# invesalius/invesalius3

Measured on AMD Instinct MI355X. Metric: Mvoxel/s segmentation + Mtriangles/s marching-cubes, 512^3 int16, 1/2/4/8 GPU, higher is better.
Workload: dtype i16; 1 GPU; configs[1]: 512x512x512 int16 per GPU, threshold(226..3071) + 26-neighbour region-grow + marching-cubes(mask@127); global_voxels=134217728, parallelism=z-slab x1, collectives=none, overlap=none

## Files before the change

### invesalius3_amd/csrc/k_mc.hip

```cpp
#include <algorithm>

#include "levels_write.h"
#include "mc_common.h"

#define MC_TABLE_QUAL static __device__ __attribute__((aligned(16))) const
#include "../../include/ivx_mc_tables.h"

typedef short short8_t __attribute__((ext_vector_type(8)));
typedef unsigned char uchar16_t __attribute__((ext_vector_type(16)));

using namespace ivx;

namespace {

template <typename T, int NISO>
__global__ __launch_bounds__(256) void k_mc_bits(const T *__restrict__ a, int64_t nrows_src, int64_t nx, int64_t ws,
                                                 double iso0, double iso1, uint8_t *__restrict__ bits0,
                                                 uint8_t *__restrict__ bits1) {
    constexpr int V = 16 / sizeof(T);
    constexpr int OB = V / 8;
    const int64_t cpr = ws * 64 / V;
    const int64_t total = nrows_src * cpr;
    const int64_t stride = (int64_t)gridDim.x * blockDim.x;
    const bool vec = (nx % V == 0) && (((uintptr_t)a & 15) == 0);
    if (vec && ws * 64 == nx) {
        const int64_t nchunk = nrows_src * (nx / V);
        typedef T vec_t __attribute__((ext_vector_type(V)));
        const vec_t *src = reinterpret_cast<const vec_t *>(a);
        for (int64_t t0 = ((int64_t)blockIdx.x * blockDim.x) * 4 + threadIdx.x; t0 < nchunk; t0 += stride * 4) {
            vec_t x[4];
#pragma unroll
            for (int u = 0; u < 4; u++) {
                const int64_t t = t0 + (int64_t)u * blockDim.x;
                if (t < nchunk) x[u] = __builtin_nontemporal_load(&src[t]);
            }
#pragma unroll
            for (int u = 0; u < 4; u++) {
                const int64_t t = t0 + (int64_t)u * blockDim.x;
                if (t >= nchunk) continue;
                unsigned m0 = 0, m1 = 0;
#pragma unroll
                for (int e = 0; e < V; e++) {
                    const double d = (double)(T)x[u][e];
                    m0 |= d >= iso0 ? (1u << e) : 0u;
                    if (NISO == 2) m1 |= d >= iso1 ? (1u << e) : 0u;
                }
                if (OB == 1) {
                    bits0[t] = (uint8_t)m0;
                    if (NISO == 2) bits1[t] = (uint8_t)m1;
                } else {
                    reinterpret_cast<uint16_t *>(bits0)[t] = (uint16_t)m0;
                    if (NISO == 2) reinterpret_cast<uint16_t *>(bits1)[t] = (uint16_t)m1;
                }
            }
        }
        return;
    }
    for (int64_t t = (int64_t)blockIdx.x * blockDim.x + threadIdx.x; t < total; t += stride) {
        const int64_t row = t / cpr, q = t - row * cpr;
        const int64_t x0 = q * V;
        unsigned m0 = 0, m1 = 0;
        if (x0 < nx) {
            const T *r = a + row * nx + x0;
            T v[V];
            if (vec) {
                if (sizeof(T) == 2) {
                    const short8_t c = *reinterpret_cast<const short8_t *>(r);
#pragma unroll
                    for (int e = 0; e < V; e++) v[e] = (T)c[e % 8];
                } else {
                    const uchar16_t c = *reinterpret_cast<const uchar16_t *>(r);
#pragma unroll
                    for (int e = 0; e < V; e++) v[e] = (T)c[e % 16];
                }
            } else {
#pragma unroll
                for (int e = 0; e < V; e++) v[e] = (x0 + e < nx) ? r[e] : (T)0;
            }
#pragma unroll
            for (int e = 0; e < V; e++) {
                const bool valid = vec || (x0 + e < nx);
                const double d = (double)v[e];
                m0 |= (valid && d >= iso0) ? (1u << e) : 0u;
                if (NISO == 2) m1 |= (valid && d >= iso1) ? (1u << e) : 0u;
            }
        }
        const int64_t ob = (row * ws * 8) + q * OB;
        if (OB == 1) {
            bits0[ob] = (uint8_t)m0;
            if (NISO == 2) bits1[ob] = (uint8_t)m1;
        } else {
            *reinterpret_cast<uint16_t *>(bits0 + ob) = (uint16_t)m0;
            if (NISO == 2) *reinterpret_cast<uint16_t *>(bits1 + ob) = (uint16_t)m1;
        }
    }
}

struct Corner8 {
    uint64_t c[8];
    uint64_t active;
};
__device__ __forceinline__ uint64_t mc_shl1(uint64_t x, uint32_t below_hi) {
    const uint32_t xl = (uint32_t)x, xh = (uint32_t)(x >> 32);
    return ((uint64_t)__builtin_amdgcn_alignbit(xh, xl, 31) << 32) | __builtin_amdgcn_alignbit(xl, below_hi, 31);
}
__device__ __forceinline__ uint64_t mc_shr1(uint64_t x, uint32_t above) {
    const uint32_t xl = (uint32_t)x, xh = (uint32_t)(x >> 32);
    return ((uint64_t)__builtin_amdgcn_alignbit(above, xh, 1) << 32) | __builtin_amdgcn_alignbit(xh, xl, 1);
}
__device__ __forceinline__ uint64_t mc_lowbits(int32_t n) {
    return n >= 64 ? ~0ull : (n <= 0 ? 0ull : ((1ull << n) - 1ull));
}
__device__ __forceinline__ Corner8 load_corners(const uint64_t *__restrict__ bits, const Geom &g, int64_t k,
                                                int64_t j, int64_t w, uint64_t pbits) {
    Corner8 r;
    const auto clampi = [](int64_t v, int64_t n) { return v >= n ? (n > 0 ? n - 1 : 0) : (v < 0 ? 0 : v); };
    const int32_t w32 = (int32_t)w, NX32 = (int32_t)g.NX, nx32 = (int32_t)g.nx, ws32 = (int32_t)g.ws;
    const uint64_t exist = mc_lowbits(NX32 - w32 * 64);
    uint64_t srcm = exist;
    if (g.pxy && w32 == 0) srcm &= ~1ull;
    srcm &= mc_lowbits(g.pxy + nx32 - w32 * 64);
    const int32_t x1 = (w32 + 1) * 64;
    const bool exist1 = x1 < NX32;
    const bool src1 = x1 - g.pxy < nx32;
    const int32_t wc = w32 >= ws32 ? (ws32 > 0 ? ws32 - 1 : 0) : w32;
    const int32_t wm = w32 - 1 >= ws32 ? (ws32 > 0 ? ws32 - 1 : 0) : (w32 - 1 < 0 ? 0 : w32 - 1);
    const int32_t wp = w32 + 1 >= ws32 ? (ws32 > 0 ? ws32 - 1 : 0) : w32 + 1;
    const int32_t ja0 = ((int32_t)g.NY - 1 - (int32_t)j) - g.pxy, ka0 = (int32_t)k - g.pb;
    const bool inner = ja0 - 1 >= 0 && ja0 < (int32_t)g.ny && ka0 >= 0 && ka0 + 1 < (int32_t)g.nz;
    if (__all(inner)) {
        const uint64_t padlo = pbits & exist & ~srcm;
        const bool use1 = exist1 && src1;
        const uint32_t nbpad = exist1 ? (uint32_t)pbits & 1u : 0u;
        const uint64_t *row = bits + (uint64_t)((uint32_t)ka0 * (uint32_t)g.ny + (uint32_t)ja0) * (uint64_t)(uint32_t)ws32;
        const uint64_t *pc = row + wc, *pa = row + (g.pxy ? wm : wp);
        const int64_t dj = -g.ws, dk = g.ny * g.ws;
        uint64_t a0[4], a1[4];
#pragma unroll
        for (int q = 0; q < 4; q++) {
            const int64_t d = ((q & 1) ? dj : 0) + ((q >> 1) ? dk : 0);
            a0[q] = pc[d];
            a1[q] = pa[d];
        }
#pragma unroll
        for (int q = 0; q < 4; q++) {
            uint64_t v0;
            uint32_t raw1;
            if (g.pxy) {
                v0 = mc_shl1(a0[q], (uint32_t)(a1[q] >> 32));
                raw1 = (uint32_t)(a0[q] >> 63);
            } else {
                v0 = a0[q];
                raw1 = (uint32_t)a1[q] & 1u;
            }
            const uint64_t lo = (v0 & srcm) | padlo;
            r.c[2 * q] = lo;
            r.c[2 * q + 1] = mc_shr1(lo, use1 ? raw1 : nbpad);
        }
    } else {
        const bool has_m = w32 - 1 >= 0 && w32 - 1 < ws32, has_c = w32 < ws32, has_p = w32 + 1 < ws32;
        uint64_t a0[4], a1[4];
        bool rin[4];
#pragma unroll
        for (int q = 0; q < 4; q++) {
            const int64_t ja = (g.NY - 1 - (j + (q & 1))) - g.pxy, ka = k + (q >> 1) - g.pb;
            rin[q] = ja >= 0 && ja < g.ny && ka >= 0 && ka < g.nz;
            const uint64_t *row = bits + (clampi(ka, g.nz) * g.ny + clampi(ja, g.ny)) * g.ws;
            a0[q] = row[wc];
            a1[q] = g.pxy ? row[wm] : row[wp];
        }
#pragma unroll
        for (int q = 0; q < 4; q++) {
            const uint64_t sc = (rin[q] && has_c) ? a0[q] : 0ull;
            uint64_t v0, raw1;
            if (g.pxy) {
                const uint64_t sm = (rin[q] && has_m) ? a1[q] : 0ull;
                v0 = (sc << 1) | (sm >> 63);
                raw1 = sc >> 63;
            } else {
                const uint64_t sp = (rin[q] && has_p) ? a1[q] : 0ull;
                v0 = sc;
                raw1 = sp & 1ull;
            }
            const uint64_t src = rin[q] ? srcm : 0ull;
            const uint64_t lo = (v0 & src) | (pbits & exist & ~src);
            const uint64_t nb = exist1 ? ((rin[q] && src1) ? raw1 : (pbits & 1ull)) : 0ull;
            r.c[2 * q] = lo;
            r.c[2 * q + 1] = (lo >> 1) | (nb << 63);
        }
    }
    uint64_t any = 0, all = ~0ull;
#pragma unroll
    for (int c = 0; c < 8; c++) {
        any |= r.c[c];
        all &= r.c[c];
    }
    r.active = any & ~all & mc_lowbits(NX32 - 1 - w32 * 64);
    return r;
}

struct McRideArgs {
    const uint16_t *reached, *inside;
    int64_t nchunks;
    uint4 *out;
    unsigned int in4, sel4;
};
template <bool RIDE, bool ALL>
__device__ __forceinline__ void mc_count_body(const uint64_t *__restrict__ bits, const Geom &g, size_t nwords, uint64_t pbits,
                                              uint16_t *__restrict__ counts, uint32_t *__restrict__ bsum, const McRideArgs &ride) {
    __shared__ uint32_t s_part[4], s_wcnt[4];
    __shared__ uint8_t s_ntri[256];
    __shared__ uint64_t s_c[256][5];
    __shared__ uint8_t s_hi[256];
    __shared__ uint16_t s_slot[256];
    const int tid = threadIdx.x, lane = tid & 63, wv = tid >> 6;
    const uint8_t ntri = MC_NTRI[tid];
    const int64_t ride_i0 = (int64_t)blockIdx.x * 1024 + tid;
    LevelsWords lw;
    if (RIDE) levels_load<ALL>(ride.reached, ride.inside, ride.nchunks, ride_i0, lw);
    auto ride_rest = [&]() {
        if (!RIDE) return;
        const int64_t stride = (int64_t)gridDim.x * 1024;
        for (int64_t i0 = ride_i0 + stride; i0 < ride.nchunks; i0 += stride) {
            LevelsWords w2;
            levels_load<ALL>(ride.reached, ride.inside, ride.nchunks, i0, w2);
            levels_store<ALL>(w2, ride.nchunks, i0, ride.out, ride.in4, ride.sel4);
        }
    };
    auto ride_store = [&]() {
#if !defined(IVX_RIDE_NO_STORES)
        if (RIDE) levels_store<ALL>(lw, ride.nchunks, ride_i0, ride.out, ride.in4, ride.sel4);
#endif
    };
    const size_t wid = (size_t)blockIdx.x * 256 + tid;
    uint64_t act = 0;
    Corner8 r;
    if (wid < nwords) {
        uint32_t k, j, w;
        mc_split_wid(g, (uint32_t)wid, k, j, w);
        r = load_corners(bits, g, (int64_t)k, (int64_t)j, (int64_t)w, pbits);
        act = r.active;
        if (!act) counts[wid] = 0;
    }
#if defined(IVX_RIDE_STORES_EARLY)
    ride_store();
#endif
    const unsigned long long am = __ballot(act != 0);
    if (lane == 0) s_wcnt[wv] = (uint32_t)__popcll(am);
    s_ntri[tid] = ntri;
    __syncthreads();
    uint32_t before = 0;
    for (int q = 0; q < wv; q++) before += s_wcnt[q];
    const uint32_t nact = s_wcnt[0] + s_wcnt[1] + s_wcnt[2] + s_wcnt[3];
#if !defined(IVX_RIDE_STORES_EARLY)
    ride_store();
#endif
#if defined(IVX_RIDE_NO_WALK)
    if (RIDE) {
        if (tid == 0) bsum[blockIdx.x] = 0;
        ride_rest();
        return;
    }
#endif
    if (!nact) {
        if (tid == 0) bsum[blockIdx.x] = 0;
        ride_rest();
        return;
    }
    if (act) {
        const uint32_t slot = before + (uint32_t)__popcll(am & ((1ull << lane) - 1ull));
        s_slot[slot] = (uint16_t)tid;
        uint32_t hi = 0;
#pragma unroll
        for (int q = 0; q < 4; q++) {
            s_c[slot][q] = r.c[2 * q];
            hi |= (uint32_t)(r.c[2 * q + 1] >> 63) << q;
        }
        s_c[slot][4] = act;
        s_hi[slot] = (uint8_t)hi;
    }
    __syncthreads();
    uint32_t n = 0;
    if ((uint32_t)tid < nact) {
        const uint64_t c0 = s_c[tid][0], c1 = s_c[tid][1], c2 = s_c[tid][2], c3 = s_c[tid][3];
        uint64_t a2 = s_c[tid][4];
        const uint32_t hi = s_hi[tid];
        while (a2) {
            const int b = __builtin_ctzll(a2);
            a2 &= a2 - 1;
            int idx;
            if (b != 63)
                idx = (int)((c0 >> b) & 3ull) | ((int)((c1 >> b) & 3ull) << 2) | ((int)((c2 >> b) & 3ull) << 4) | ((int)((c3 >> b) & 3ull) << 6);
            else
                idx = (int)(c0 >> 63) | ((int)(hi & 1u) << 1) | ((int)(c1 >> 63) << 2) | ((int)(hi >> 1 & 1u) << 3) | ((int)(c2 >> 63) << 4) |
                      ((int)(hi >> 2 & 1u) << 5) | ((int)(c3 >> 63) << 6) | ((int)(hi >> 3 & 1u) << 7);
            n += s_ntri[idx];
        }
        counts[(size_t)blockIdx.x * 256 + s_slot[tid]] = (uint16_t)n;
    }
    uint32_t s = n;
#pragma unroll
    for (int o = 32; o > 0; o >>= 1) s += __shfl_xor(s, o, 64);
    if (lane == 0) s_part[wv] = s;
    __syncthreads();
    if (tid == 0) bsum[blockIdx.x] = s_part[0] + s_part[1] + s_part[2] + s_part[3];
    ride_rest();
}
__global__ __launch_bounds__(256) void k_mc_count(const uint64_t *__restrict__ bits, Geom g, size_t nwords,
                                                  uint64_t pbits, uint16_t *__restrict__ counts,
                                                  uint32_t *__restrict__ bsum) {
    mc_count_body<false, false>(bits, g, nwords, pbits, counts, bsum, McRideArgs{});
}
template <bool ALL>
__global__ __launch_bounds__(256) void k_mc_count_write(const uint64_t *__restrict__ bits, Geom g, size_t nwords, uint64_t pbits,
                                                        uint16_t *__restrict__ counts, uint32_t *__restrict__ bsum, McRideArgs ride,
                                                        ApplyWhen when) {
    if (apply_when_skips(when)) return;
    mc_count_body<true, ALL>(bits, g, nwords, pbits, counts, bsum, ride);
}

__global__ __launch_bounds__(1024) void k_mc_scan(const uint32_t *__restrict__ bsum, size_t n,
                                                  uint64_t *__restrict__ boff, uint32_t *mb, uint32_t seq) {
    __shared__ uint64_t s_wave[16];
    __shared__ uint64_t s_carry;
    __shared__ uint32_t s_tot[64], s_exc[64];
    constexpr int RND = 4;
    const int lane = threadIdx.x & 63, wv = threadIdx.x >> 6;
    const size_t base = (size_t)blockIdx.x * (1024 * 4 * RND);
    uint64_t pre = 0;
    {
        const uint4 *b4 = reinterpret_cast<const uint4 *>(bsum);
        const size_t n4 = base / 4;
        uint64_t p0 = 0, p1 = 0, p2 = 0, p3 = 0;
        size_t i = threadIdx.x;
        for (; i + 3 * 1024 < n4; i += 4 * 1024) {
            const uint4 a = b4[i], b = b4[i + 1024], c = b4[i + 2048], d = b4[i + 3072];
            p0 += (uint64_t)a.x + a.y + a.z + a.w;
            p1 += (uint64_t)b.x + b.y + b.z + b.w;
            p2 += (uint64_t)c.x + c.y + c.z + c.w;
            p3 += (uint64_t)d.x + d.y + d.z + d.w;
        }
        for (; i < n4; i += 1024) {
            const uint4 a = b4[i];
            p0 += (uint64_t)a.x + a.y + a.z + a.w;
        }
        pre = p0 + p1 + p2 + p3;
    }
#pragma unroll
    for (int o = 32; o > 0; o >>= 1) pre += __shfl_xor(pre, o, 64);
    if (lane == 0) s_wave[wv] = pre;
    const bool al16 = ((uintptr_t)bsum & 15) == 0 && ((uintptr_t)boff & 15) == 0;
    uint32_t v[RND][4], inc[RND];
#pragma unroll
    for (int r = 0; r < RND; r++) {
        const size_t i0 = base + (size_t)r * 4096 + (size_t)threadIdx.x * 4;
        if (al16 && i0 + 3 < n) {
            const uint4 a = *reinterpret_cast<const uint4 *>(bsum + i0);
            v[r][0] = a.x; v[r][1] = a.y; v[r][2] = a.z; v[r][3] = a.w;
        } else {
#pragma unroll
            for (int q = 0; q < 4; q++) v[r][q] = i0 + q < n ? bsum[i0 + q] : 0u;
        }
    }
#pragma unroll
    for (int r = 0; r < RND; r++) {
        inc[r] = v[r][0] + v[r][1] + v[r][2] + v[r][3];
#pragma unroll
        for (int o = 1; o < 64; o <<= 1) {
            const uint32_t t = __shfl_up(inc[r], o, 64);
            if (lane >= o) inc[r] += t;
        }
        if (lane == 63) s_tot[r * 16 + wv] = inc[r];
    }
    __syncthreads();
    if (wv == 0) {
        const uint32_t t = s_tot[lane];
        uint32_t e = t;
#pragma unroll
        for (int o = 1; o < 64; o <<= 1) {
            const uint32_t u = __shfl_up(e, o, 64);
            if (lane >= o) e += u;
        }
        s_exc[lane] = e - t;
        uint64_t c = 0;
        for (int q = 0; q < 16; q++) c += s_wave[q];
        if (lane == 0) s_carry = c;
        if (lane == 63 && base + 1024 * 4 * RND >= n) {
            const uint64_t total = c + e;
            boff[n] = total;
            if (mb) {
                mb[0] = (uint32_t)total;
                mb[1] = (uint32_t)(total >> 32);
                __threadfence_system();
                __hip_atomic_store(&mb[63], seq, __ATOMIC_RELEASE, __HIP_MEMORY_SCOPE_SYSTEM);
            }
        }
    }
    __syncthreads();
    const uint64_t carry = s_carry;
#pragma unroll
    for (int r = 0; r < RND; r++) {
        const size_t i0 = base + (size_t)r * 4096 + (size_t)threadIdx.x * 4;
        const uint32_t lanesum = v[r][0] + v[r][1] + v[r][2] + v[r][3];
        const uint64_t o0 = carry + (uint64_t)(s_exc[r * 16 + wv] + inc[r] - lanesum);
        const uint64_t o1 = o0 + v[r][0], o2 = o1 + v[r][1], o3 = o2 + v[r][2];
        if (al16 && i0 + 3 < n) {
            typedef unsigned long long u64x2_t __attribute__((ext_vector_type(2)));
            u64x2_t *d = reinterpret_cast<u64x2_t *>(boff + i0);
            d[0] = u64x2_t{o0, o1};
            d[1] = u64x2_t{o2, o3};
        } else {
            if (i0 < n) boff[i0] = o0;
            if (i0 + 1 < n) boff[i0 + 1] = o1;
            if (i0 + 2 < n) boff[i0 + 2] = o2;
            if (i0 + 3 < n) boff[i0 + 3] = o3;
        }
    }
}

constexpr int MCL_CHUNK = 256;
constexpr int MCL_CELLS = 2048;
__device__ __forceinline__ uint32_t mcl_wave_scan(uint32_t v) {
    v += (uint32_t)__builtin_amdgcn_update_dpp(0, (int)v, 0x111, 0xf, 0xf, false);
    v += (uint32_t)__builtin_amdgcn_update_dpp(0, (int)v, 0x112, 0xf, 0xf, false);
    v += (uint32_t)__builtin_amdgcn_update_dpp(0, (int)v, 0x114, 0xf, 0xf, false);
    v += (uint32_t)__builtin_amdgcn_update_dpp(0, (int)v, 0x118, 0xf, 0xf, false);
    v += (uint32_t)__builtin_amdgcn_update_dpp(0, (int)v, 0x142, 0xa, 0xf, false);
    v += (uint32_t)__builtin_amdgcn_update_dpp(0, (int)v, 0x143, 0xc, 0xf, false);
    return v;
}
__global__ __launch_bounds__(256) void k_mc_list(const uint64_t *__restrict__ bits, Geom g, size_t nwords, uint64_t pbits,
                                                 const uint16_t *__restrict__ counts, const uint64_t *__restrict__ boff,
                                                 uint64_t *__restrict__ list, uint64_t max_tris) {
    __shared__ uint32_t s_wave[4], s_part[2][4];
    __shared__ uint8_t s_ntri[256];
    __shared__ uint64_t s_c[4][256];
    __shared__ uint8_t s_hi[256];
    __shared__ uint64_t s_pre[256];
    __shared__ uint16_t s_cell[MCL_CELLS];
    const int tid = threadIdx.x, lane = tid & 63, wv = tid >> 6;
    const uint8_t ntri = MC_NTRI[tid];
    const size_t wid0 = (size_t)blockIdx.x * 256;
    const uint32_t n = wid0 + tid < nwords ? (uint32_t)counts[wid0 + tid] : 0u;
    const uint64_t pos0 = boff[blockIdx.x];
    if (boff[blockIdx.x + 1] == pos0 || pos0 >= max_tris) return;
    uint64_t a2 = 0;
    if (n) {
        uint32_t k, j, w;
        mc_split_wid(g, (uint32_t)(wid0 + tid), k, j, w);
        const Corner8 r = load_corners(bits, g, (int64_t)k, (int64_t)j, (int64_t)w, pbits);
        a2 = r.active;
        uint32_t hi = 0;
#pragma unroll
        for (int q = 0; q < 4; q++) {
            s_c[q][tid] = r.c[2 * q];
            hi |= (uint32_t)(r.c[2 * q + 1] >> 63) << q;
        }
        s_hi[tid] = (uint8_t)hi;
        s_pre[tid] = ((uint64_t)k << 48) | ((uint64_t)j << 32) | ((uint64_t)w << 17);
    }
    const uint32_t pc = (uint32_t)__popcll(a2);
    const uint32_t inc = mcl_wave_scan(pc);
    if (lane == 63) s_wave[wv] = inc;
    s_ntri[tid] = ntri;
    __syncthreads();
    uint32_t ci = inc - pc;
    for (int q = 0; q < wv; q++) ci += s_wave[q];
    const uint32_t ncell = s_wave[0] + s_wave[1] + s_wave[2] + s_wave[3];
    uint64_t P = pos0;
    int par = 0;
    for (uint32_t sb = 0; sb < ncell; sb += MCL_CELLS) {
        const uint32_t se = sb + MCL_CELLS < ncell ? sb + MCL_CELLS : ncell;
        while (a2 && ci < se) {
            const int b = __builtin_ctzll(a2);
            a2 &= a2 - 1;
            s_cell[ci - sb] = (uint16_t)((tid << 6) | b);
            ci++;
        }
        __syncthreads();
        for (uint32_t cb = sb; cb < se; cb += MCL_CHUNK) {
            const uint32_t c = cb + tid;
            uint32_t nt = 0;
            uint64_t d0 = 0;
            if (c < se) {
                const uint32_t rec = s_cell[c - sb], sl = rec >> 6;
                const int b = (int)(rec & 63u);
                const uint64_t c0 = s_c[0][sl], c1 = s_c[1][sl], c2 = s_c[2][sl], c3 = s_c[3][sl];
                int idx;
                if (b != 63) {
                    idx = (int)((c0 >> b) & 3ull) | ((int)((c1 >> b) & 3ull) << 2) | ((int)((c2 >> b) & 3ull) << 4) | ((int)((c3 >> b) & 3ull) << 6);
                } else {
                    const uint32_t hi = s_hi[sl];
                    idx = (int)(c0 >> 63) | ((int)(hi & 1u) << 1) | ((int)(c1 >> 63) << 2) | ((int)(hi >> 1 & 1u) << 3) | ((int)(c2 >> 63) << 4) |
                          ((int)(hi >> 2 & 1u) << 5) | ((int)(c3 >> 63) << 6) | ((int)(hi >> 3 & 1u) << 7);
                }
                nt = s_ntri[idx];
                d0 = s_pre[sl] | ((uint64_t)b << 11) | ((uint64_t)idx << 3);
            }
            const uint32_t ti = mcl_wave_scan(nt);
            if (lane == 63) s_part[par][wv] = ti;
            __syncthreads();
            uint32_t off = ti - nt;
            for (int q = 0; q < wv; q++) off += s_part[par][q];
            const uint32_t tot = s_part[par][0] + s_part[par][1] + s_part[par][2] + s_part[par][3];
            const uint64_t p0 = P + off;
#pragma unroll
            for (uint32_t t = 0; t < MC_MAX_TRI; t++)
                if (t < nt && p0 + t < max_tris) list[p0 + t] = d0 | t;
            P += tot;
            if (P >= max_tris) return;
            par ^= 1;
        }
    }
}

template <typename T, bool LEVELS>
__device__ __forceinline__ void mc_triangle(const T *__restrict__ a, const Geom &g, const McLevels &lv, double iso,
                                            const uint8_t *s_tri, const int *s_e0, const int *s_e1, const int *s_ec, int32_t k,
                                            int32_t j, int32_t i, int idx, int rel, float *o) {
    const int32_t ka = k - (int32_t)g.pb, ja = ((int32_t)g.NY - 1 - j) - (int32_t)g.pxy;
    const int32_t ia = i - (int32_t)g.pxy;
    const bool fast = ka >= 0 && ka + 1 < (int32_t)g.nz && ja - 1 >= 0 && ja < (int32_t)g.ny && ia >= 0 &&
                      ia + 1 < (int32_t)g.nx;
    double s0[3], s1[3];
    int ec[3];
#pragma unroll
    for (int v = 0; v < 3; v++) ec[v] = s_tri[idx * 15 + 3 * rel + v];
    double ttl[3];
    if (LEVELS) {
#pragma unroll
        for (int v = 0; v < 3; v++) {
            const int c = s_ec[ec[v]];
            const int ax = c & 3, bx = (c >> 2) & 1, by = (c >> 3) & 1, bz = (c >> 4) & 1;
            const int lo = bx + 2 * by + 4 * bz;
            const bool in0 = (idx >> lo) & 1, in1 = (idx >> (lo + (1 << ax))) & 1;
            const int32_t kk = k + bz + (in1 && ax == 2), jj = j + by + (in1 && ax == 1), ii = i + bx + (in1 && ax == 0);
            const int64_t sk = kk - (int32_t)g.pb, sj = ((int32_t)g.NY - 1 - jj) - (int32_t)g.pxy, si = ii - (int32_t)g.pxy;
            const uint64_t wsel = lv.sel[(sk * g.ny + sj) * g.ws + (si >> 6)];
            ttl[v] = lv.tt[(in0 ? 2 : 0) + (int)((wsel >> (si & 63)) & 1ull)];
            ec[v] = c;
        }
    } else if (fast) {
        const T *cell = a + ((int64_t)ka * g.ny + ja) * g.nx + ia;
#pragma unroll
        for (int v = 0; v < 3; v++) {
            s0[v] = (double)cell[s_e0[ec[v]]];
            s1[v] = (double)cell[s_e1[ec[v]]];
        }
#pragma unroll
        for (int v = 0; v < 3; v++) ec[v] = s_ec[ec[v]];
    } else {
#pragma unroll
        for (int v = 0; v < 3; v++) {
            const int c = s_ec[ec[v]];
            const int ax = c & 3, bx = (c >> 2) & 1, by = (c >> 3) & 1, bz = (c >> 4) & 1;
            s0[v] = mc_at(a, g, k + bz, j + by, i + bx);
            s1[v] = mc_at(a, g, k + bz + (ax == 2), j + by + (ax == 1), i + bx + (ax == 0));
            ec[v] = c;
        }
    }
#pragma unroll
    for (int v = 0; v < 3; v++) {
        const int ax = ec[v] & 3, bx = (ec[v] >> 2) & 1, by = (ec[v] >> 3) & 1, bz = (ec[v] >> 4) & 1;
        const double tt = LEVELS ? ttl[v] : (iso - s0[v]) / (s1[v] - s0[v]);
        double p0 = (double)(i + bx - (int32_t)g.pxy);
        double p1 = (double)(j + by - (int32_t)g.yoff);
        double p2 = (double)(k + bz + g.zoff);
        if (ax == 0) p0 += tt;
        else if (ax == 1) p1 += tt;
        else p2 += tt;
        o[3 * v + 0] = (float)(g.sx * p0);
        o[3 * v + 1] = (float)(g.sy * p1);
        o[3 * v + 2] = (float)(g.sz * p2);
    }
}

template <typename T, bool LEVELS>
__global__ __launch_bounds__(256) void k_mc_emit(const T *__restrict__ a, Geom g, double iso0, double iso1,
                                                 const uint64_t *__restrict__ split_dev,
                                                 const uint64_t *__restrict__ total_dev,
                                                 const uint64_t *__restrict__ list, uint64_t cap,
                                                 float *__restrict__ tris, McLevels lv) {
    __shared__ __attribute__((aligned(16))) uint8_t s_tri[256 * 15];
    __shared__ __attribute__((aligned(16))) float s_out[256 * 9];
    const int tid = threadIdx.x;
    const uint64_t total = *total_dev, split = *split_dev;
    const uint64_t ntris = total < cap ? total : cap;
    const uint64_t T0 = (uint64_t)blockIdx.x * 256;
    if (T0 >= ntris) return;
#pragma unroll
    for (int q = 0; q < 4; q++)
        if (q * 256 + tid < 960) ((uint32_t *)s_tri)[q * 256 + tid] = ((const uint32_t *)&MC_TRI[0][0])[q * 256 + tid];
    const uint64_t T_ = T0 + tid;
    const double iso = T_ < split ? iso0 : iso1;
    __shared__ int s_e0[12], s_e1[12], s_ec[12];
    const int plane32 = (int)(g.ny * g.nx), nx32 = (int)g.nx;
    if (tid < 12) {
        int ax, bx, by, bz;
        edge_decode(tid, ax, bx, by, bz);
        const int o0 = bz * plane32 - by * nx32 + bx;
        s_e0[tid] = o0;
        s_e1[tid] = o0 + (ax == 2 ? plane32 : (ax == 1 ? -nx32 : 1));
        s_ec[tid] = ax | (bx << 2) | (by << 3) | (bz << 4);
    }
    const bool live = T_ < ntris;
    const uint64_t d = live ? list[T_] : 0ull;
    __syncthreads();
    if (live) {
        const int b = (int)(d >> 11) & 63, idx = (int)(d >> 3) & 255, rel = (int)d & 7;
        const uint32_t w = (uint32_t)(d >> 17) & 0x7fffu;
        const int32_t k = (int32_t)(d >> 48), j = (int32_t)((d >> 32) & 0xffffull);
        mc_triangle<T, LEVELS>(a, g, lv, iso, s_tri, s_e0, s_e1, s_ec, k, j, (int32_t)w * 64 + b, idx, rel, s_out + tid * 9);
    }
    __syncthreads();
    const uint32_t nt_chunk = ntris - T0 < 256 ? (uint32_t)(ntris - T0) : 256u;
    float *dst = tris + T0 * 9;
    if (nt_chunk == 256 && ((uintptr_t)tris & 15) == 0) {
        typedef float float4_t __attribute__((ext_vector_type(4)));
        float4_t *d4 = (float4_t *)dst;
        const float4_t *s4 = (const float4_t *)s_out;
        __builtin_nontemporal_store(s4[tid], &d4[tid]);
        __builtin_nontemporal_store(s4[tid + 256], &d4[tid + 256]);
        if (tid < 64) __builtin_nontemporal_store(s4[tid + 512], &d4[tid + 512]);
    } else {
        for (uint32_t f = tid; f < nt_chunk * 9; f += 256) dst[f] = s_out[f];
    }
}

template <typename T>
static int run_bits(const ivx_mc_params *p, const Geom &g, const Scratch &s, const void *a, uint8_t *b0, double iso0,
                    double iso1, hipStream_t st) {
    constexpr int V = 16 / sizeof(T);
    const int64_t nrows_src = g.nz * g.ny;
    const int64_t total = nrows_src * (g.ws * 64 / V);
    if (total == 0) return IVX_OK;
    const int64_t blocks = ivx::cdiv(total, 256 * 4);
    const int grid = (int)(blocks < 1 ? 1 : (blocks < 16384 ? blocks : 16384));
    uint8_t *b1 = b0 + s.bits_words * 8;
    if (p->niso == 2)
        hipLaunchKernelGGL((k_mc_bits<T, 2>), dim3(grid), dim3(256), 0, st, (const T *)a, nrows_src, g.nx, g.ws,
                           iso0, iso1, b0, b1);
    else
        hipLaunchKernelGGL((k_mc_bits<T, 1>), dim3(grid), dim3(256), 0, st, (const T *)a, nrows_src, g.nx, g.ws,
                           iso0, 0.0, b0, b0);
    IVX_LAUNCH_CHECK();
    return IVX_OK;
}

template <typename T>
static int run_emit(const ivx_mc_params *p, const Geom &g, const Scratch &s, const void *a, const char *scratch,
                    float *tris, int64_t max_tris, hipStream_t st, const McLevels *lv) {
    const uint64_t *boff = (const uint64_t *)(scratch + s.off_boff);
    void *d_list;
    int rc = ws_get_s(WS_MCLIST, st, (size_t)max_tris * 8 + 64, &d_list);
    if (rc) return rc;
    const size_t nb = s.nblocks * (size_t)p->niso;
    if (!mc_pieces().list_ready(scratch, d_list, max_tris))
        if ((rc = mc_queue_list(p, g, s, scratch, d_list, max_tris, st))) return rc;
    if (lv)
        hipLaunchKernelGGL((k_mc_emit<T, true>), dim3((unsigned)ivx::cdiv(max_tris, (int64_t)256)), dim3(256), 0, st, (const T *)a, g,
                           p->iso[0], p->iso[1], boff + (p->niso == 2 ? s.nblocks : nb), boff + nb, (const uint64_t *)d_list,
                           (uint64_t)max_tris, tris, *lv);
    else
        hipLaunchKernelGGL((k_mc_emit<T, false>), dim3((unsigned)ivx::cdiv(max_tris, (int64_t)256)), dim3(256), 0, st, (const T *)a, g,
                           p->iso[0], p->iso[1], boff + (p->niso == 2 ? s.nblocks : nb), boff + nb, (const uint64_t *)d_list,
                           (uint64_t)max_tris, tris, McLevels{nullptr, 0.0, 0.0, 0.0, {0.0, 0.0, 0.0, 0.0}});
    IVX_LAUNCH_CHECK();
    return IVX_OK;
}

}

namespace ivx {

int mc_piece_layout(const ivx_mc_params *p, Geom *g, Scratch *s, bool *empty) {
    int rc = make_geom(p, g);
    if (rc) return rc;
    *s = make_scratch(*g, p->niso);
    *empty = s->nwords == 0;
    if (*empty) return IVX_OK;
    IVX_REQUIRE(s->nblocks * (size_t)p->niso < 0x7fffffffull, IVX_EINVAL, "mc: piece too large for one launch");
    IVX_REQUIRE(s->nwords < 0xffffffffull, IVX_EINVAL, "mc: piece too large for 32-bit cell-word ids");
    return IVX_OK;
}

int mc_inside_planes(const ivx_mc_params *p, const Geom &g, const Scratch &s, const void *a, void *dst, double iso0, double iso1,
                     hipStream_t st) {
    return MC_BY_DTYPE(p->dtype, run_bits, p, g, s, a, (uint8_t *)dst, iso0, iso1, st);
}

int mc_queue_list(const ivx_mc_params *p, const Geom &g, const Scratch &s, const void *scratch_, void *d_list, int64_t max_tris,
                  hipStream_t st) {
    const char *scratch = (const char *)scratch_;
    const uint64_t *boff = (const uint64_t *)(scratch + s.off_boff);
    for (int q = 0; q < p->niso; q++) {
        const uint64_t *bits = mc_bits_ptr(scratch, s, q);
        const uint16_t *counts = (const uint16_t *)(scratch + s.off_counts) + (size_t)q * s.nwords;
        hipLaunchKernelGGL(k_mc_list, dim3((unsigned)s.nblocks), dim3(256), 0, st, bits, g, s.nwords, pad_bits(p, q), counts,
                           boff + (size_t)q * s.nblocks, (uint64_t *)d_list, (uint64_t)max_tris);
        IVX_LAUNCH_CHECK();
    }
    return IVX_OK;
}

int mc_upload_piece(const ivx_mc_params *p, const void *a, const int64_t strides[3], void **d_a, void **d_scr) {
    size_t sb;
    int rc = ivx_dev_mc_scratch_bytes(p, &sb);
    if (rc) return rc;
    const size_t isz = dtype_size(p->dtype);
    const int64_t shape[3] = {p->nz, p->ny, p->nx};
    if ((rc = ws_get(WS_IN, (size_t)p->nz * p->ny * p->nx * isz, d_a))) return rc;
    if ((rc = ws_get(WS_AUX0, sb, d_scr))) return rc;
    return upload_strided(*d_a, a, shape, strides, isz, WS_IN);
}

}

extern "C" int ivx_mc_split_word_ids(const ivx_mc_params *p, const uint32_t *wid, size_t n, uint32_t *k, uint32_t *j, uint32_t *w) {
    Geom g;
    int rc = make_geom(p, &g);
    if (rc) return rc;
    for (size_t i = 0; i < n; i++) mc_split_wid(g, wid[i], k[i], j[i], w[i]);
    return IVX_OK;
}

extern "C" int ivx_dev_mc_scratch_bytes(const ivx_mc_params *p, size_t *nbytes) {
    Geom g;
    int rc = make_geom(p, &g);
    if (rc) return rc;
    *nbytes = make_scratch(g, p->niso).total;
    return IVX_OK;
}

static int mc_read_total(const ivx_mc_params *p, const Scratch &s, void *scratch_, int64_t *ntris, hipStream_t st) {
    char *scratch = (char *)scratch_;
    int rc;
    uint64_t *boff = (uint64_t *)(scratch + s.off_boff);
    const size_t nb = s.nblocks * (size_t)p->niso;
    uint32_t seq, tw[2];
    if (p->niso == 2) {
        uint32_t seq0, t0[2];
        if ((rc = ivx::mailbox_publish(boff + s.nblocks, 2, st, &seq0))) return rc;
        if ((rc = ivx::mailbox_wait(seq0, st, t0, 2))) return rc;
        mc_pieces().set_split(scratch_, ((uint64_t)t0[1] << 32) | t0[0]);
    }
    if ((rc = ivx::mailbox_publish(boff + nb, 2, st, &seq))) return rc;
    if ((rc = ivx::mailbox_wait(seq, st, tw, 2))) return rc;
    *ntris = (int64_t)(((uint64_t)tw[1] << 32) | tw[0]);
    return IVX_OK;
}

static int mc_read_total_early(const ivx_mc_params *p, const Scratch &s, void *scratch_, int64_t *ntris, hipStream_t st) {
    const uint32_t seq = p->niso == 1 ? mc_pieces().total_seq(scratch_) : 0u;
    if (seq) {
        uint32_t tw[2];
        int got = 0;
        const int rc = ivx::mailbox_wait_reserved(seq, st, tw, 2, &got);
        if (rc) return rc;
        if (got) {
            *ntris = (int64_t)(((uint64_t)tw[1] << 32) | tw[0]);
            return IVX_OK;
        }
    }
    return mc_read_total(p, s, scratch_, ntris, st);
}

static void mc_count_record(void *scratch_, const uint64_t *inside_bits) { mc_pieces().begin_count(scratch_, inside_bits); }
static int mc_count_launch(const ivx_mc_params *p, const Geom &g, const Scratch &s, void *scratch_, hipStream_t st) {
    char *scratch = (char *)scratch_;
    uint32_t *bsum = (uint32_t *)(scratch + s.off_bsum);
    for (int q = 0; q < p->niso; q++) {
        const uint64_t *bits = mc_bits_ptr(scratch, s, q);
        uint16_t *counts = (uint16_t *)(scratch + s.off_counts) + (size_t)q * s.nwords;
        hipLaunchKernelGGL(k_mc_count, dim3((unsigned)s.nblocks), dim3(256), 0, st, bits, g, s.nwords, pad_bits(p, q),
                           counts, bsum + (size_t)q * s.nblocks);
        IVX_LAUNCH_CHECK();
    }
    return IVX_OK;
}
static int mc_count_scan(const ivx_mc_params *p, const Scratch &s, void *scratch_, hipStream_t st) {
    char *scratch = (char *)scratch_;
    uint32_t *bsum = (uint32_t *)(scratch + s.off_bsum);
    uint64_t *boff = (uint64_t *)(scratch + s.off_boff);
    const size_t nb = s.nblocks * (size_t)p->niso;
    uint32_t *mb = nullptr, seq = 0;
    if (p->niso == 1) {
        int rc = ivx::mailbox_reserve(&mb, &seq);
        if (rc) return rc;
        mc_pieces().set_total_seq(scratch_, seq);
    }
    hipLaunchKernelGGL(k_mc_scan, dim3((unsigned)std::max<size_t>(1, (nb + 16383) / 16384)), dim3(1024), 0, st, bsum, nb, boff, mb,
                       seq);
    IVX_LAUNCH_CHECK();
    return IVX_OK;
}

static int mc_count_impl(const ivx_mc_params *p, const void *a, const uint64_t *inside_bits, void *scratch_, int64_t *ntris,
                         void *stream) {
    Geom g;
    Scratch s;
    bool empty;
    int rc = mc_piece_layout(p, &g, &s, &empty);
    if (rc) return rc;
    IVX_REQUIRE(!inside_bits || p->niso == 1, IVX_EINVAL, "mc_count_bits: one iso-value only");
    if (ntris) *ntris = 0;
    if (empty) return IVX_OK;
    IVX_REQUIRE(a || inside_bits, IVX_EINVAL, "mc_count: neither voxels nor an inside plane");
    char *scratch = (char *)scratch_;
    hipStream_t st = S(stream);
    mc_count_record(scratch_, inside_bits);
    if (!inside_bits && (rc = mc_inside_planes(p, g, s, a, scratch + s.off_bits, p->iso[0], p->iso[1], st))) return rc;
    if ((rc = mc_count_launch(p, g, s, scratch_, st))) return rc;
    if ((rc = mc_count_scan(p, s, scratch_, st))) return rc;
    return ntris ? mc_read_total_early(p, s, scratch_, ntris, st) : IVX_OK;
}

bool ivx::mc_ride_ok(const ivx_mc_params *p, const void *scratch, int64_t dz, int64_t dy, int64_t dx) {
    Geom g;
    Scratch s;
    bool empty;
    if (!p || !scratch || mc_piece_layout(p, &g, &s, &empty) != IVX_OK || empty) return false;
    return p->niso == 1 && p->ny == dy && p->nx == dx && p->nz <= dz;
}
void ivx::mc_ride_begin(void *scratch, const uint64_t *inside_bits) { mc_count_record(scratch, inside_bits); }
int ivx::mc_ride_launch(const ivx_mc_params *p, void *scratch_, const uint64_t *reached, const uint64_t *inside, int64_t nchunks,
                        uint8_t *mask, int v_in, int v_sel, bool all, const ApplyWhen &when, hipStream_t st) {
    Geom g;
    Scratch s;
    bool empty;
    int rc = mc_piece_layout(p, &g, &s, &empty);
    if (rc) return rc;
    IVX_REQUIRE(!empty && p->niso == 1 && nchunks > 0, IVX_EINVAL, "mc_ride: an empty piece or volume, or two iso-values");
    char *scratch = (char *)scratch_;
    const McRideArgs ride = {(const uint16_t *)reached, (const uint16_t *)inside, nchunks, (uint4 *)mask, 0x01010101u * (uint8_t)v_in,
                             0x01010101u * (uint8_t)v_sel};
    auto k = all ? k_mc_count_write<true> : k_mc_count_write<false>;
    hipLaunchKernelGGL(k, dim3((unsigned)s.nblocks), dim3(256), 0, st, mc_bits_ptr(scratch, s, 0), g, s.nwords, pad_bits(p, 0),
                       (uint16_t *)(scratch + s.off_counts), (uint32_t *)(scratch + s.off_bsum), ride, when);
    IVX_LAUNCH_CHECK();
    return IVX_OK;
}
int ivx::mc_ride_scan(const ivx_mc_params *p, void *scratch, hipStream_t st) {
    Geom g;
    Scratch s;
    bool empty;
    int rc = mc_piece_layout(p, &g, &s, &empty);
    if (rc) return rc;
    return mc_count_scan(p, s, scratch, st);
}

extern "C" int ivx_dev_mc_count(const ivx_mc_params *p, const void *a, void *scratch_, int64_t *ntris, void *stream) {
    return mc_count_impl(p, a, nullptr, scratch_, ntris, stream);
}
extern "C" int ivx_dev_mc_count_async(const ivx_mc_params *p, const void *a, void *scratch_, void *stream) {
    return mc_count_impl(p, a, nullptr, scratch_, nullptr, stream);
}
extern "C" int ivx_dev_mc_total(const ivx_mc_params *p, void *scratch_, int64_t *ntris, void *stream) {
    Geom g;
    Scratch s;
    bool empty;
    int rc = mc_piece_layout(p, &g, &s, &empty);
    if (rc) return rc;
    *ntris = 0;
    return empty ? IVX_OK : mc_read_total(p, s, scratch_, ntris, S(stream));
}
extern "C" int ivx_dev_mc_total_early(const ivx_mc_params *p, void *scratch_, int64_t *ntris, void *stream) {
    Geom g;
    Scratch s;
    bool empty;
    int rc = mc_piece_layout(p, &g, &s, &empty);
    if (rc) return rc;
    *ntris = 0;
    return empty ? IVX_OK : mc_read_total_early(p, s, scratch_, ntris, S(stream));
}

extern "C" int ivx_dev_mc_count_bits(const ivx_mc_params *p, const uint64_t *inside_bits, void *scratch_, int64_t *ntris,
                                     void *stream) {
    return mc_count_impl(p, nullptr, inside_bits, scratch_, ntris, stream);
}
extern "C" int ivx_dev_mc_count_bits_async(const ivx_mc_params *p, const uint64_t *inside_bits, void *scratch_, void *stream) {
    return mc_count_impl(p, nullptr, inside_bits, scratch_, nullptr, stream);
}

extern "C" int ivx_dev_mc_emit(const ivx_mc_params *p, const void *a, const void *scratch, float *tris,
                               int64_t max_tris, void *stream) {
    Geom g;
    Scratch s;
    bool empty;
    int rc = mc_piece_layout(p, &g, &s, &empty);
    if (rc) return rc;
    if (empty || max_tris <= 0) return IVX_OK;
    return MC_BY_DTYPE(p->dtype, run_emit, p, g, s, a, (const char *)scratch, tris, max_tris, S(stream), nullptr);
}

extern "C" int ivx_dev_mc_emit_levels(const ivx_mc_params *p, const void *scratch, const uint64_t *sel_bits, double v_out,
                                      double v_in, double v_sel, float *tris, int64_t max_tris, void *stream) {
    Geom g;
    Scratch s;
    bool empty;
    int rc = mc_piece_layout(p, &g, &s, &empty);
    if (rc) return rc;
    IVX_REQUIRE(p->dtype == IVX_U8 && p->niso == 1 && sel_bits, IVX_EINVAL, "mc_emit_levels: uint8 mask, one iso-value");
    IVX_REQUIRE(v_out < p->iso[0] && v_in >= p->iso[0] && v_sel >= p->iso[0] && (double)p->pad_value == v_out, IVX_EINVAL,
                "mc_emit_levels: v_out must lie below the iso-value and equal the padding value, v_in and v_sel at or above it");
    if (empty || max_tris <= 0) return IVX_OK;
    const McLevels lv = make_levels(sel_bits, p->iso[0], v_out, v_in, v_sel);
    return run_emit<uint8_t>(p, g, s, nullptr, (const char *)scratch, tris, max_tris, S(stream), &lv);
}

extern "C" int ivx_dev_mc_list(const ivx_mc_params *p, const void *scratch, int64_t max_tris, void *stream) {
    Geom g;
    Scratch s;
    bool empty;
    int rc = mc_piece_layout(p, &g, &s, &empty);
    if (rc) return rc;
    if (empty || max_tris <= 0) return IVX_OK;
    hipStream_t st = S(stream);
    void *d_list;
    if ((rc = ws_get_s(WS_MCLIST, st, (size_t)max_tris * 8 + 64, &d_list))) return rc;
    if ((rc = mc_queue_list(p, g, s, scratch, d_list, max_tris, st))) return rc;
    mc_pieces().list_built(scratch, d_list, max_tris);
    return IVX_OK;
}

extern "C" int ivx_marching_cubes(const ivx_mc_params *p, const void *a, const int64_t strides[3], float *tris,
                                  int64_t max_tris, int64_t *ntris) {
    HostCallGuard host_guard__;
    void *d_a, *d_scr;
    int rc = mc_upload_piece(p, a, strides, &d_a, &d_scr);
    if (rc) return rc;
    int64_t cnt = 0;
    if ((rc = ivx_dev_mc_count(p, d_a, d_scr, &cnt, nullptr))) return rc;
    *ntris = cnt;
    if (!tris || cnt == 0) return IVX_OK;
    IVX_REQUIRE(max_tris >= cnt, IVX_ERANGE, "mc: output buffer holds %lld triangles, %lld needed", (long long)max_tris,
                (long long)cnt);
    void *d_tris;
    if ((rc = ws_get(WS_OUT, (size_t)cnt * 36, &d_tris))) return rc;
    if ((rc = ivx_dev_mc_emit(p, d_a, d_scr, (float *)d_tris, cnt, nullptr))) return rc;
    IVX_HIP(hipMemcpy(tris, d_tris, (size_t)cnt * 36, hipMemcpyDeviceToHost));
    return IVX_OK;
}

static uint64_t g_mc_begin_epoch = 0;
static int64_t g_mc_begin_count = 0;
extern "C" int ivx_marching_cubes_begin(const ivx_mc_params *p, const void *a, const int64_t strides[3], int64_t *ntris) {
    HostCallGuard host_guard__;
    IVX_REQUIRE(p && a && ntris, IVX_EINVAL, "marching_cubes_begin: null argument");
    g_mc_begin_epoch = 0;
    void *d_a, *d_scr;
    int rc = mc_upload_piece(p, a, strides, &d_a, &d_scr);
    if (rc) return rc;
    int64_t cnt = 0;
    if ((rc = ivx_dev_mc_count(p, d_a, d_scr, &cnt, nullptr))) return rc;
    *ntris = cnt;
    if (cnt) {
        void *d_tris;
        if ((rc = ws_get(WS_OUT, (size_t)cnt * 36, &d_tris))) return rc;
        if ((rc = ivx_dev_mc_emit(p, d_a, d_scr, (float *)d_tris, cnt, nullptr))) return rc;
    }
    g_mc_begin_epoch = host_epoch();
    g_mc_begin_count = cnt;
    return IVX_OK;
}
extern "C" int ivx_marching_cubes_fetch(float *tris, int64_t ntris) {
    ivx::HostCallGuard host_guard__;
    IVX_REQUIRE(g_mc_begin_epoch != 0 && host_epoch() == g_mc_begin_epoch + 1 && ntris == g_mc_begin_count, IVX_EINVAL,
                "marching_cubes_fetch: not the call right behind ivx_marching_cubes_begin (or another count): take ivx_marching_cubes");
    g_mc_begin_epoch = 0;
    if (ntris == 0) return IVX_OK;
    IVX_REQUIRE(tris, IVX_EINVAL, "marching_cubes_fetch: null buffer");
    void *d_tris;
    int rc;
    if ((rc = ws_get(WS_OUT, (size_t)ntris * 36, &d_tris))) return rc;
    return copy_d2h(tris, d_tris, (size_t)ntris * 36);
}
```

Measured before the change: 445,700 Mvoxel/s.

## Make marching-cubes emit kernel persistent with prefetched descriptors and 32-bit level lookups

The triangle emit kernel becomes a grid-stride persistent kernel sized to resident occupancy. Each block loads the triangle table into shared memory once and prefetches the next chunk's descriptor while it stores the current chunk. The levels path now reads the selector mask as 32-bit halves, uses 32-bit index arithmetic when the volume is small, and caches the four tt values in shared memory. Alignment and index width become template parameters. The change also adds environment overrides and debug macros, and makes an extra occupancy query on the first call.

```diff
diff --git a/invesalius3_amd/csrc/k_mc.hip b/invesalius3_amd/csrc/k_mc.hip
--- a/invesalius3_amd/csrc/k_mc.hip
+++ b/invesalius3_amd/csrc/k_mc.hip
@@ -1,4 +1,5 @@
 #include <algorithm>
+#include <type_traits>
 
 #include "levels_write.h"
 #include "mc_common.h"
@@ -514,10 +515,10 @@
     }
 }
 
-template <typename T, bool LEVELS>
+template <typename T, bool LEVELS, bool WIDE>
 __device__ __forceinline__ void mc_triangle(const T *__restrict__ a, const Geom &g, const McLevels &lv, double iso,
-                                            const uint8_t *s_tri, const int *s_e0, const int *s_e1, const int *s_ec, int32_t k,
-                                            int32_t j, int32_t i, int idx, int rel, float *o) {
+                                            const uint8_t *s_tri, const int *s_e0, const int *s_e1, const int *s_ec,
+                                            const double *s_tt, int32_t k, int32_t j, int32_t i, int idx, int rel, float *o) {
     const int32_t ka = k - (int32_t)g.pb, ja = ((int32_t)g.NY - 1 - j) - (int32_t)g.pxy;
     const int32_t ia = i - (int32_t)g.pxy;
     const bool fast = ka >= 0 && ka + 1 < (int32_t)g.nz && ja - 1 >= 0 && ja < (int32_t)g.ny && ia >= 0 &&
@@ -535,9 +536,15 @@
             const int lo = bx + 2 * by + 4 * bz;
             const bool in0 = (idx >> lo) & 1, in1 = (idx >> (lo + (1 << ax))) & 1;
             const int32_t kk = k + bz + (in1 && ax == 2), jj = j + by + (in1 && ax == 1), ii = i + bx + (in1 && ax == 0);
-            const int64_t sk = kk - (int32_t)g.pb, sj = ((int32_t)g.NY - 1 - jj) - (int32_t)g.pxy, si = ii - (int32_t)g.pxy;
-            const uint64_t wsel = lv.sel[(sk * g.ny + sj) * g.ws + (si >> 6)];
-            ttl[v] = lv.tt[(in0 ? 2 : 0) + (int)((wsel >> (si & 63)) & 1ull)];
+            const int32_t sk = kk - (int32_t)g.pb, sj = ((int32_t)g.NY - 1 - jj) - (int32_t)g.pxy, si = ii - (int32_t)g.pxy;
+            const int64_t half = WIDE ? (((int64_t)sk * g.ny + sj) * g.ws + (si >> 6)) * 2 + ((si >> 5) & 1)
+                                      : (int64_t)(((sk * (int32_t)g.ny + sj) * (int32_t)g.ws + (si >> 6)) * 2 + ((si >> 5) & 1));
+#if IVX_EMIT_CONST_SEL
+            const uint32_t wsel = 0u;
+#else
+            const uint32_t wsel = ((const uint32_t *)lv.sel)[half];
+#endif
+            ttl[v] = s_tt[(in0 ? 2 : 0) + (int)((wsel >> (si & 31)) & 1u)];
             ec[v] = c;
         }
     } else if (fast) {
@@ -575,25 +582,38 @@
     }
 }
 
-template <typename T, bool LEVELS>
+__device__ __forceinline__ uint64_t emit_desc(const uint64_t *__restrict__ list, uint64_t ntris, uint64_t c, int tid) {
+    const uint64_t t = c * 256 + tid;
+    return list[t < ntris ? t : ntris - 1];
+}
+
+template <typename T, bool LEVELS, bool ALIGNED, bool WIDE>
 __global__ __launch_bounds__(256) void k_mc_emit(const T *__restrict__ a, Geom g, double iso0, double iso1,
                                                  const uint64_t *__restrict__ split_dev,
                                                  const uint64_t *__restrict__ total_dev,
                                                  const uint64_t *__restrict__ list, uint64_t cap,
                                                  float *__restrict__ tris, McLevels lv) {
-    __shared__ __attribute__((aligned(16))) uint8_t s_tri[256 * 15];
     __shared__ __attribute__((aligned(16))) float s_out[256 * 9];
+    __shared__ int s_e0[12], s_e1[12], s_ec[12];
+    __shared__ double s_tt[4];
     const int tid = threadIdx.x;
     const uint64_t total = *total_dev, split = *split_dev;
     const uint64_t ntris = total < cap ? total : cap;
-    const uint64_t T0 = (uint64_t)blockIdx.x * 256;
-    if (T0 >= ntris) return;
-#pragma unroll
-    for (int q = 0; q < 4; q++)
-        if (q * 256 + tid < 960) ((uint32_t *)s_tri)[q * 256 + tid] = ((const uint32_t *)&MC_TRI[0][0])[q * 256 + tid];
-    const uint64_t T_ = T0 + tid;
-    const double iso = T_ < split ? iso0 : iso1;
-    __shared__ int s_e0[12], s_e1[12], s_ec[12];
+    const uint64_t nchunks = (ntris + 255) >> 8, G = gridDim.x;
+    uint64_t c = blockIdx.x;
+    if (c >= nchunks) return;
+    uint64_t d = emit_desc(list, ntris, c, tid);
+#if IVX_EMIT_TABLE_GLOBAL
+    const uint8_t *s_tri = &MC_TRI[0][0];
+#else
+    __shared__ __attribute__((aligned(16))) uint8_t s_tri[256 * 15];
+    const uint32_t *tri32 = (const uint32_t *)&MC_TRI[0][0];
+    const uint32_t t0 = tri32[tid], t1 = tri32[256 + tid], t2 = tri32[512 + tid];
+    if (tid < 192) ((uint32_t *)s_tri)[768 + tid] = tri32[768 + tid];
+    ((uint32_t *)s_tri)[tid] = t0;
+    ((uint32_t *)s_tri)[256 + tid] = t1;
+    ((uint32_t *)s_tri)[512 + tid] = t2;
+#endif
     const int plane32 = (int)(g.ny * g.nx), nx32 = (int)g.nx;
     if (tid < 12) {
         int ax, bx, by, bz;
@@ -603,27 +623,42 @@
         s_e1[tid] = o0 + (ax == 2 ? plane32 : (ax == 1 ? -nx32 : 1));
         s_ec[tid] = ax | (bx << 2) | (by << 3) | (bz << 4);
     }
-    const bool live = T_ < ntris;
-    const uint64_t d = live ? list[T_] : 0ull;
+    if (LEVELS && tid < 4) s_tt[tid] = lv.tt[tid];
     __syncthreads();
-    if (live) {
-        const int b = (int)(d >> 11) & 63, idx = (int)(d >> 3) & 255, rel = (int)d & 7;
-        const uint32_t w = (uint32_t)(d >> 17) & 0x7fffu;
-        const int32_t k = (int32_t)(d >> 48), j = (int32_t)((d >> 32) & 0xffffull);
-        mc_triangle<T, LEVELS>(a, g, lv, iso, s_tri, s_e0, s_e1, s_ec, k, j, (int32_t)w * 64 + b, idx, rel, s_out + tid * 9);
-    }
-    __syncthreads();
-    const uint32_t nt_chunk = ntris - T0 < 256 ? (uint32_t)(ntris - T0) : 256u;
-    float *dst = tris + T0 * 9;
-    if (nt_chunk == 256 && ((uintptr_t)tris & 15) == 0) {
-        typedef float float4_t __attribute__((ext_vector_type(4)));
-        float4_t *d4 = (float4_t *)dst;
-        const float4_t *s4 = (const float4_t *)s_out;
-        __builtin_nontemporal_store(s4[tid], &d4[tid]);
-        __builtin_nontemporal_store(s4[tid + 256], &d4[tid + 256]);
-        if (tid < 64) __builtin_nontemporal_store(s4[tid + 512], &d4[tid + 512]);
-    } else {
-        for (uint32_t f = tid; f < nt_chunk * 9; f += 256) dst[f] = s_out[f];
+#if IVX_EMIT_NO_STORES
+    const bool stores = cap == ~0ull;
+#else
+    const bool stores = true;
+#endif
+    for (;;) {
+        const uint64_t T0 = c * 256;
+        if (T0 + tid < ntris) {
+            const int b = (int)(d >> 11) & 63, idx = (int)(d >> 3) & 255, rel = (int)d & 7;
+            const uint32_t w = (uint32_t)(d >> 17) & 0x7fffu;
+            const int32_t k = (int32_t)(d >> 48), j = (int32_t)((d >> 32) & 0xffffull);
+            mc_triangle<T, LEVELS, WIDE>(a, g, lv, T0 + tid < split ? iso0 : iso1, s_tri, s_e0, s_e1, s_ec, s_tt, k, j,
+                                         (int32_t)w * 64 + b, idx, rel, s_out + tid * 9);
+        }
+        const uint64_t dn = emit_desc(list, ntris, c + G, tid);
+        __syncthreads();
+        const uint32_t nt_chunk = ntris - T0 < 256 ? (uint32_t)(ntris - T0) : 256u;
+        float *dst = tris + T0 * 9;
+        if (!ALIGNED || nt_chunk < 256) {
+            if (stores)
+                for (uint32_t f = tid; f < nt_chunk * 9; f += 256) dst[f] = s_out[f];
+            if (ALIGNED) break;
+        } else if (stores) {
+            typedef float float4_t __attribute__((ext_vector_type(4)));
+            float4_t *d4 = (float4_t *)dst;
+            const float4_t *s4 = (const float4_t *)s_out;
+            __builtin_nontemporal_store(s4[tid], &d4[tid]);
+            __builtin_nontemporal_store(s4[tid + 256], &d4[tid + 256]);
+            if (tid < 64) __builtin_nontemporal_store(s4[tid + 512], &d4[tid + 512]);
+        }
+        c += G;
+        if (c >= nchunks) break;
+        d = dn;
+        __syncthreads();
     }
 }
 
@@ -647,6 +682,40 @@
     return IVX_OK;
 }
 
+constexpr int64_t EMIT_RESIDENT_MIN = 32;
+template <typename T, bool LEVELS, bool ALIGNED, bool WIDE>
+static int emit_grid(int64_t chunks, unsigned *grid) {
+    static const int64_t resident = []() {
+        int dev = 0, cus = 0, per_cu = 0;
+        if (hipGetDevice(&dev) != hipSuccess || hipDeviceGetAttribute(&cus, hipDeviceAttributeMultiprocessorCount, dev) != hipSuccess ||
+            hipOccupancyMaxActiveBlocksPerMultiprocessor(&per_cu, k_mc_emit<T, LEVELS, ALIGNED, WIDE>, 256, 0) != hipSuccess)
+            return (int64_t)0;
+        return (int64_t)cus * per_cu;
+    }();
+    IVX_REQUIRE(resident > 0, IVX_EHIP, "mc: the runtime reports no occupancy for the emit kernel");
+    int64_t resident_min = EMIT_RESIDENT_MIN;
+    if (const char *e = getenv("IVX_MC_EMIT_RESIDENT_MIN"))
+        if (atoll(e) > 0) resident_min = atoll(e);
+    int64_t wgs = chunks >= resident_min * resident ? resident : chunks;
+    if (const char *e = getenv("IVX_MC_EMIT_WGS"))
+        if (atoll(e) > 0) wgs = atoll(e);
+    *grid = (unsigned)(chunks < wgs ? chunks : wgs);
+    return IVX_OK;
+}
+
+template <typename T, bool LEVELS, bool ALIGNED, bool WIDE>
+static int launch_emit(const ivx_mc_params *p, const Geom &g, const Scratch &s, const void *a, const uint64_t *boff,
+                       const void *d_list, float *tris, int64_t max_tris, hipStream_t st, const McLevels &lv) {
+    unsigned grid;
+    int rc = emit_grid<T, LEVELS, ALIGNED, WIDE>(ivx::cdiv(max_tris, (int64_t)256), &grid);
+    if (rc) return rc;
+    const size_t nb = s.nblocks * (size_t)p->niso;
+    hipLaunchKernelGGL((k_mc_emit<T, LEVELS, ALIGNED, WIDE>), dim3(grid), dim3(256), 0, st, (const T *)a, g, p->iso[0], p->iso[1],
+                       boff + (p->niso == 2 ? s.nblocks : nb), boff + nb, (const uint64_t *)d_list, (uint64_t)max_tris, tris, lv);
+    IVX_LAUNCH_CHECK();
+    return IVX_OK;
+}
+
 template <typename T>
 static int run_emit(const ivx_mc_params *p, const Geom &g, const Scratch &s, const void *a, const char *scratch,
                     float *tris, int64_t max_tris, hipStream_t st, const McLevels *lv) {
@@ -654,19 +723,24 @@
     void *d_list;
     int rc = ws_get_s(WS_MCLIST, st, (size_t)max_tris * 8 + 64, &d_list);
     if (rc) return rc;
-    const size_t nb = s.nblocks * (size_t)p->niso;
     if (!mc_pieces().list_ready(scratch, d_list, max_tris))
         if ((rc = mc_queue_list(p, g, s, scratch, d_list, max_tris, st))) return rc;
-    if (lv)
-        hipLaunchKernelGGL((k_mc_emit<T, true>), dim3((unsigned)ivx::cdiv(max_tris, (int64_t)256)), dim3(256), 0, st, (const T *)a, g,
-                           p->iso[0], p->iso[1], boff + (p->niso == 2 ? s.nblocks : nb), boff + nb, (const uint64_t *)d_list,
-                           (uint64_t)max_tris, tris, *lv);
-    else
-        hipLaunchKernelGGL((k_mc_emit<T, false>), dim3((unsigned)ivx::cdiv(max_tris, (int64_t)256)), dim3(256), 0, st, (const T *)a, g,
-                           p->iso[0], p->iso[1], boff + (p->niso == 2 ? s.nblocks : nb), boff + nb, (const uint64_t *)d_list,
-                           (uint64_t)max_tris, tris, McLevels{nullptr, 0.0, 0.0, 0.0, {0.0, 0.0, 0.0, 0.0}});
-    IVX_LAUNCH_CHECK();
-    return IVX_OK;
+    const bool aligned = ((uintptr_t)tris & 15) == 0;
+    if (lv) {
+        if constexpr (std::is_same<T, uint8_t>::value) {
+            const bool wide = g.nz * g.ny * g.ws >= (1ll << 30);
+            if (wide)
+                return aligned ? launch_emit<T, true, true, true>(p, g, s, a, boff, d_list, tris, max_tris, st, *lv)
+                               : launch_emit<T, true, false, true>(p, g, s, a, boff, d_list, tris, max_tris, st, *lv);
+            return aligned ? launch_emit<T, true, true, false>(p, g, s, a, boff, d_list, tris, max_tris, st, *lv)
+                           : launch_emit<T, true, false, false>(p, g, s, a, boff, d_list, tris, max_tris, st, *lv);
+        } else {
+            IVX_REQUIRE(false, IVX_EINVAL, "mc: the levels form takes a uint8 mask");
+        }
+    }
+    const McLevels none{nullptr, 0.0, 0.0, 0.0, {0.0, 0.0, 0.0, 0.0}};
+    return aligned ? launch_emit<T, false, true, false>(p, g, s, a, boff, d_list, tris, max_tris, st, none)
+                   : launch_emit<T, false, false, false>(p, g, s, a, boff, d_list, tris, max_tris, st, none);
 }
 
 }
```

Result: faster. 455,700 Mvoxel/s, median of 6 (+2.2%).
